# ACMMM2021-Anonymous/video-graph-ssl

Hardware: AMD Instinct MI355X
Metric: pretrain_clips_per_sec (higher is better)
Workload: dtype bf16x6 (fp32 tensors; conv products as 6 bf16 MFMAs on hi/mid/lo splits = fp32-grade, fp32 accumulate; everything else fp32)

## Files before the change

### include/gca_hip.h

```cpp
#ifndef GCA_HIP_H
#define GCA_HIP_H

#include <stdint.h>

#ifdef __cplusplus
extern "C" {
#endif

#define GCA_OK 0
#define GCA_EINVAL (-1)
#define GCA_ELAUNCH (-2)

int gca_version(void);

int gca_conv_halo_occupancy(int tm, int tn, int math, int64_t lds_bytes);

int gca_set_conv_math(int mode);
int gca_get_conv_math(void);

typedef struct {
  int32_t N, C, D, H, W;
  int32_t K;
  int32_t kd, kh, kw;
  int32_t sd, sh, sw;
// ... 64 lines not shown
                    float* save_mean, float* save_invstd, float* scale, float* shift, void* stream);
int gca_conv_fwd_slabs(const gca_conv_geom* g, const void* x, const float* wpack, const int32_t* table, void* ws,
                       int32_t* out_splits, void* stream);
int gca_bn_train_fwd_slabs(const float* slabs, int64_t splits, double count, const float* gamma, const float* beta, float eps,
                           float momentum, float* running_mean, float* running_var, int64_t* num_batches_tracked,
                           float* save_mean, float* save_invstd, float* scale, float* shift, float* y, const float* residual,
                           int relu, int64_t N, int64_t C, int64_t SP, float* z, int64_t z_batch_stride, void* stream);
int gca_bn_train_fwd(const float* stat_sum, const float* stat_sq, int64_t P, int64_t C, double count,
                     const float* gamma, const float* beta, float eps, float momentum,
                     float* running_mean, float* running_var, int64_t* num_batches_tracked,
                     float* save_mean, float* save_invstd, float* scale, float* shift,
                     const void* x, const void* residual, int relu, int64_t N, int64_t SP, void* z,
                     int64_t z_batch_stride, int act_f16, void* stream);
int gca_bn_fold_eval(const float* gamma, const float* beta, const float* running_mean,
                     const float* running_var, float eps, int64_t C, float* scale, float* shift, void* stream);
int gca_bn_apply(const void* x, const float* scale, const float* shift, const void* residual,
                 int relu, int64_t N, int64_t C, int64_t SP, void* z, int64_t z_batch_stride, int act_f16, void* stream);
int64_t gca_bn_bwd_ws_bytes(int64_t N, int64_t C, int64_t SP);
int gca_bn_bwd(const void* dz_in, const void* z, const void* x, const float* gamma,
               const float* save_mean, const float* save_invstd, int relu,
               int64_t N, int64_t C, int64_t SP, void* dx, float* dgamma, float* dbeta,
               void* dres, int dres_accumulate, int64_t z_batch_stride ,
               const float* scale, const float* shift, void* ws, int act_f16, void* stream);

typedef struct {
  int32_t N, C, D, H, W;
  int32_t kd, kh, kw, sd, sh, sw, pd, ph, pw;
  int32_t OD, OH, OW;
} gca_pool_geom;
int gca_maxpool3d_fwd(const gca_pool_geom* g, const void* x, void* y, int32_t* argmax, const float* scale,
                      const float* shift, int act_f16, void* stream);
int gca_maxpool3d_bwd(const gca_pool_geom* g, const void* dy, const int32_t* argmax, void* dx,
                      int accumulate, int act_f16, void* stream);
int gca_avgpool3d_fwd(const gca_pool_geom* g, const float* x, float* y, void* stream);
int gca_avgpool3d_bwd(const gca_pool_geom* g, const float* dy, float* dx, int accumulate, void* stream);
int gca_wavgpool_fwd(const void* x, const float* wt, float norm, int64_t NC, int64_t D, int64_t HW,
                     float* y, int x_f16, void* stream);
int gca_wavgpool_bwd(const float* dy, const float* wt, float norm, int64_t NC, int64_t D, int64_t HW,
                     void* dx, int x_f16, void* stream);

int gca_relu_fwd(const float* x, int64_t n, float* y, void* stream);
int gca_relu_bwd(const float* dy, const float* y, int64_t n, float* dx, void* stream);
int gca_l2norm_fwd(const float* x, int64_t rows, int64_t dim, float eps, float* y, float* inv_norm, void* stream);
int gca_l2norm_bwd(const float* dy, const float* y, const float* inv_norm, int64_t rows, int64_t dim,
                   float* dx, void* stream);
int gca_negcos_fwd_bwd(const float* p, const float* z, int64_t rows, int64_t dim, float scale,
                       float* loss, int accumulate, float* dp, void* stream);

int64_t gca_infonce_ws_bytes(int64_t b, int64_t K);
int gca_moco_logits_fwd(const float* q, const float* k, const float* queue, int64_t b, int64_t K,
                        int64_t D, float inv_T, float* logits, float* row_lse, int32_t* rank_ge, float* loss,
                        void* ws, uint32_t* sync_counter, void* stream);
int gca_nce_softmax_loss_fwd(const float* logits, int64_t b, int64_t ncol, const float* row_lse_in,
                             float* row_lse_out, float* loss, void* stream);
int gca_nce_softmax_loss_bwd(const float* logits, const float* row_lse, int64_t b, int64_t ncol,
                             const float* gscale_dev, float gscale_host, float* dlogits, void* stream);
int gca_moco_logits_bwd(const float* dlogits, const float* logits, const float* row_lse,
                        const float* gscale_dev, float gscale_host,
                        const float* k, const float* queue, int64_t b, int64_t K, int64_t D, float inv_T,
                        int64_t ov_start, const int64_t* ov_start_dev ,
                        int64_t ov_n, const float* ov_rows, float* dq, void* ws, void* stream);
int gca_rank_ge(const float* output, const int64_t* target, int64_t b, int64_t ncol, int32_t* rank_ge, void* stream);
int gca_queue_enqueue(float* queue, int64_t K, int64_t D, const float* keys, int64_t n, int64_t ptr,
                      const int64_t* ptr_dev, float* saved_rows, void* stream);
int gca_queue_advance(int64_t* ptr_dev, int64_t n, int64_t K, void* stream);

// ... 39 lines not shown
```

### video-graph-ssl_amd/_hip.py

```python
import ctypes as C
import os

import torch

_HERE = os.path.dirname(os.path.abspath(__file__))
LIB_PATH = os.environ.get('GCA_LIB_PATH') or os.path.join(_HERE, 'libgca_hip.so')


class HipLibraryMissing(RuntimeError):
    pass


if not os.path.exists(LIB_PATH):
    raise HipLibraryMissing(
        'libgca_hip.so is not built (%s). Run ./build_hip.sh or __graft_entry__.build(); there is no '
        'CPU fallback for the product path.' % LIB_PATH)
lib = C.CDLL(LIB_PATH)

c_i32, c_i64, c_f32, c_f64, c_vp = C.c_int32, C.c_int64, C.c_float, C.c_double, C.c_void_p


class ConvGeom(C.Structure):
    _fields_ = [(n, c_i32) for n in ('N', 'C', 'D', 'H', 'W', 'K', 'kd', 'kh', 'kw', 'sd', 'sh', 'sw',
                                     'pd', 'ph', 'pw', 'OD', 'OH', 'OW')] + [('x_batch_stride', c_i64)] + \
# ... 12 lines not shown
SIGNATURES = {
    'gca_version': (c_i32, []),
    'gca_conv_halo_occupancy': (c_i32, [c_i32, c_i32, c_i32, c_i64]),
    'gca_set_conv_math': (c_i32, [c_i32]),
    'gca_get_conv_math': (c_i32, []),
    'gca_conv_pack_elems': (c_i64, [_GP, c_i32]),
    'gca_conv_pack': (c_i32, [_GP, c_i32, c_vp, c_vp, c_vp]),
    'gca_conv_table_rows': (c_i64, [_GP, c_i32]),
    'gca_conv_table_build_host': (c_i32, [_GP, c_i32, c_vp]),
    'gca_conv_fwd_stat_parts': (c_i64, [_GP]),
    'gca_conv_kernel_cfg': (c_i32, [_GP, c_i32, c_vp]),
    'gca_conv_pack_layout': (c_i64, [_GP, c_i32]),
    'gca_conv_fwd_ws_bytes': (c_i64, [_GP]),
    'gca_conv_fwd': (c_i32, [_GP, c_vp, c_vp, c_vp, c_vp, c_vp, c_vp, c_vp, c_vp, c_vp]),
    'gca_conv_dgrad_ws_bytes': (c_i64, [_GP]),
    'gca_conv_dgrad': (c_i32, [_GP, c_vp, c_vp, c_vp, c_vp, c_i32, c_vp, c_vp]),
    'gca_conv_wgrad_cfg': (c_i32, [_GP, c_vp]),
    'gca_conv_wgrad_ws_bytes': (c_i64, [_GP]),
    'gca_conv_wgrad': (c_i32, [_GP, c_vp, c_vp, c_vp, c_vp, c_i32, c_vp, c_vp]),
    'gca_bias_grad': (c_i32, [c_vp, c_i64, c_i64, c_i64, c_vp, c_i32, c_vp]),
    'gca_bn_stats': (c_i32, [c_vp, c_i64, c_i64, c_i64, c_vp, c_vp, c_vp, c_i32, c_vp]),
    'gca_bn_stats_parts': (c_i64, [c_i64, c_i64, c_i64]),
    'gca_bn_finalize': (c_i32, [c_vp, c_vp, c_i64, c_i64, c_f64, c_vp, c_vp, c_f32, c_f32, c_vp, c_vp, c_vp,
                                c_vp, c_vp, c_vp, c_vp, c_vp]),
    'gca_bn_train_fwd': (c_i32, [c_vp, c_vp, c_i64, c_i64, c_f64, c_vp, c_vp, c_f32, c_f32, c_vp, c_vp, c_vp,
                                 c_vp, c_vp, c_vp, c_vp, c_vp, c_vp, c_i32, c_i64, c_i64, c_vp, c_i64, c_i32, c_vp]),
    'gca_bn_fold_eval': (c_i32, [c_vp, c_vp, c_vp, c_vp, c_f32, c_i64, c_vp, c_vp, c_vp]),
    'gca_bn_apply': (c_i32, [c_vp, c_vp, c_vp, c_vp, c_i32, c_i64, c_i64, c_i64, c_vp, c_i64, c_i32, c_vp]),
    'gca_bn_bwd_ws_bytes': (c_i64, [c_i64, c_i64, c_i64]),
    'gca_bn_bwd': (c_i32, [c_vp, c_vp, c_vp, c_vp, c_vp, c_vp, c_i32, c_i64, c_i64, c_i64, c_vp, c_vp, c_vp,
                           c_vp, c_i32, c_i64, c_vp, c_vp, c_vp, c_i32, c_vp]),
    'gca_maxpool3d_fwd': (c_i32, [_PP, c_vp, c_vp, c_vp, c_vp, c_vp, c_i32, c_vp]),
    'gca_maxpool3d_bwd': (c_i32, [_PP, c_vp, c_vp, c_vp, c_i32, c_i32, c_vp]),
    'gca_avgpool3d_fwd': (c_i32, [_PP, c_vp, c_vp, c_vp]),
    'gca_avgpool3d_bwd': (c_i32, [_PP, c_vp, c_vp, c_i32, c_vp]),
    'gca_wavgpool_fwd': (c_i32, [c_vp, c_vp, c_f32, c_i64, c_i64, c_i64, c_vp, c_i32, c_vp]),
    'gca_wavgpool_bwd': (c_i32, [c_vp, c_vp, c_f32, c_i64, c_i64, c_i64, c_vp, c_i32, c_vp]),
    'gca_relu_fwd': (c_i32, [c_vp, c_i64, c_vp, c_vp]),
    'gca_relu_bwd': (c_i32, [c_vp, c_vp, c_i64, c_vp, c_vp]),
    'gca_l2norm_fwd': (c_i32, [c_vp, c_i64, c_i64, c_f32, c_vp, c_vp, c_vp]),
    'gca_l2norm_bwd': (c_i32, [c_vp, c_vp, c_vp, c_i64, c_i64, c_vp, c_vp]),
    'gca_negcos_fwd_bwd': (c_i32, [c_vp, c_vp, c_i64, c_i64, c_f32, c_vp, c_i32, c_vp, c_vp]),
    'gca_infonce_ws_bytes': (c_i64, [c_i64, c_i64]),
    'gca_moco_logits_fwd': (c_i32, [c_vp, c_vp, c_vp, c_i64, c_i64, c_i64, c_f32, c_vp, c_vp, c_vp, c_vp, c_vp, c_vp, c_vp]),
    'gca_nce_softmax_loss_fwd': (c_i32, [c_vp, c_i64, c_i64, c_vp, c_vp, c_vp, c_vp]),
    'gca_nce_softmax_loss_bwd': (c_i32, [c_vp, c_vp, c_i64, c_i64, c_vp, c_f32, c_vp, c_vp]),
    'gca_moco_logits_bwd': (c_i32, [c_vp, c_vp, c_vp, c_vp, c_f32, c_vp, c_vp, c_i64, c_i64, c_i64, c_f32,
                                    c_i64, c_vp, c_i64, c_vp, c_vp, c_vp, c_vp]),
    'gca_queue_enqueue': (c_i32, [c_vp, c_i64, c_i64, c_vp, c_i64, c_i64, c_vp, c_vp, c_vp]),
    'gca_queue_advance': (c_i32, [c_vp, c_i64, c_i64, c_vp]),
    'gca_graph_gram_ws_bytes': (c_i64, [c_i64, c_i64, c_i64, c_i64]),
    'gca_graph_adj_fwd': (c_i32, [c_vp, c_vp, c_i64, c_i64, c_i64, c_i64, c_i32, c_f32, c_f32, c_vp, c_vp,
                                  c_vp, c_vp, c_vp, c_vp]),
    'gca_graph_adj_bwd': (c_i32, [c_vp, c_vp, c_vp, c_vp, c_vp, c_vp, c_i64, c_i64, c_i64, c_i64, c_i32, c_f32,
                                  c_f32, c_vp, c_vp, c_vp]),
    'gca_graph_gcn_fwd': (c_i32, [c_vp, c_vp, c_i64, c_i64, c_i64, c_i64, c_vp, c_vp]),
    'gca_graph_gcn_bwd_ws_bytes': (c_i64, [c_i64, c_i64, c_i64, c_i64]),
    'gca_graph_gcn_bwd': (c_i32, [c_vp, c_vp, c_vp, c_i64, c_i64, c_i64, c_i64, c_vp, c_vp, c_vp, c_vp]),
    'gca_ema_update': (c_i32, [c_vp, c_vp, c_i64, c_f32, c_vp]),
    'gca_sgd_step': (c_i32, [c_vp, c_vp, c_vp, c_i64, c_vp, c_vp, c_f32, c_f32, c_i32, c_i32, c_vp, c_vp]),
    'gca_grad_clip_ws_bytes': (c_i64, []),
    'gca_grad_clip_coef': (c_i32, [c_vp, c_i64, c_f32, c_vp, c_vp, c_vp]),
    'gca_conv_wgrad_partial': (c_i32, [_GP, c_vp, c_vp, c_vp, c_vp, c_vp, c_vp, c_vp, c_vp]),
    'gca_conv_xf_ok': (c_i32, [_GP]),
    'gca_conv_fwd_xf': (c_i32, [_GP, c_vp, c_vp, c_vp, c_vp, c_vp, c_vp, c_vp, c_vp, c_vp, c_vp, c_vp]),
    'gca_conv_wgrad_xf': (c_i32, [_GP, c_vp, c_vp, c_vp, c_vp, c_vp, c_vp, c_i32, c_vp, c_vp]),
# ... 65 lines not shown
```

### video-graph-ssl_amd/csrc/bn.hip

```cpp
#include "gca_common.h"

namespace {

constexpr int STAT_CHUNK = 8192;
constexpr int MAX_PARTS = 256;
constexpr long long BN_SMALL_ELEMS = 32768;

__host__ __device__ inline long long stats_parts(long long N, long long C, long long SP) {
  long long p = (N * SP + STAT_CHUNK - 1) / STAT_CHUNK;
  if (p < 1) p = 1;
  if (p > MAX_PARTS) p = MAX_PARTS;
  return p;
}

template <typename T, int MODE, int VEC>
__global__ __launch_bounds__(256) void bn_reduce_kernel(
    const T* __restrict__ a, const T* __restrict__ z, const T* __restrict__ x,
    const float* __restrict__ mean, const float* __restrict__ invstd, int relu,
    long long N, long long C, long long SP, long long zs, int P, float* __restrict__ out0,
    float* __restrict__ out1, const float* __restrict__ scale, const float* __restrict__ shift) {
  typedef gca_act<T> A_;
  __shared__ double sh[4];
  const int c = blockIdx.y, part = blockIdx.x;
  const float rsc = relu == 2 ? scale[c] : 0.f, rsf = relu == 2 ? shift[c] : 0.f;
// ... 588 lines not shown
                    (((uintptr_t)dz_in | (uintptr_t)z | (uintptr_t)x | (uintptr_t)dx | (uintptr_t)dres) % 16 == 0);
    if (s4)
      hipLaunchKernelGGL((bn_bwd_small_kernel<T, 4>), dim3((unsigned)C), dim3(256), 0, st, dz_in, z, x, gamma, save_mean, save_invstd,
                         relu, (int)N, (int)C, (int)SP, zs, dx, dgamma, dbeta, dres, dres_accumulate, scale, shift);
    else
      hipLaunchKernelGGL((bn_bwd_small_kernel<T, 1>), dim3((unsigned)C), dim3(256), 0, st, dz_in, z, x, gamma, save_mean, save_invstd,
                         relu, (int)N, (int)C, (int)SP, zs, dx, dgamma, dbeta, dres, dres_accumulate, scale, shift);
    return gca_launch_status();
  }
  const int P = (int)stats_parts(N, C, SP);
  float* p0 = reinterpret_cast<float*>(ws);
  float* p1 = p0 + (long long)C * P;
  float* coef = p1 + (long long)C * P;
  if ((SP % 4 == 0) && (zs % 4 == 0) && (((uintptr_t)dz_in | (uintptr_t)z | (uintptr_t)x) % 16 == 0))
    hipLaunchKernelGGL((bn_reduce_kernel<T, 1, 4>), dim3(P, (unsigned)C), dim3(256), 0, st, dz_in, z, x, save_mean,
                       save_invstd, relu, (long long)N, (long long)C, (long long)SP, zs, P, p0, p1, scale, shift);
  else
    hipLaunchKernelGGL((bn_reduce_kernel<T, 1, 1>), dim3(P, (unsigned)C), dim3(256), 0, st, dz_in, z, x, save_mean,
                       save_invstd, relu, (long long)N, (long long)C, (long long)SP, zs, P, p0, p1, scale, shift);
  hipLaunchKernelGGL(bn_bwd_finalize_kernel, dim3((unsigned)C), dim3(256), 0, st, p0, p1, P, (double)N * (double)SP,
                     gamma, save_invstd, dgamma, dbeta, coef, (long long)C);
  const long long total = (long long)N * C * SP;
  const bool v4 = (SP % 4 == 0) && (zs % 4 == 0) &&
                  (((uintptr_t)dz_in | (uintptr_t)z | (uintptr_t)x | (uintptr_t)dx | (uintptr_t)dres) % 16 == 0);
  if (v4)
    hipLaunchKernelGGL((bn_bwd_apply_kernel<T, 4>), dim3(ew_grid(total, 4)), dim3(256), 0, st, dz_in, z, x, save_mean,
                       save_invstd, coef, relu, total, (long long)C, (long long)SP, zs, dx, dres, dres_accumulate, scale, shift);
  else
    hipLaunchKernelGGL((bn_bwd_apply_kernel<T, 1>), dim3(ew_grid(total, 1)), dim3(256), 0, st, dz_in, z, x, save_mean,
                       save_invstd, coef, relu, total, (long long)C, (long long)SP, zs, dx, dres, dres_accumulate, scale, shift);
  return gca_launch_status();
}

extern "C" {

int64_t gca_bn_stats_parts(int64_t N, int64_t C, int64_t SP) { return stats_parts(N, C, SP); }


int gca_bn_finalize(const float* stat_sum, const float* stat_sq, int64_t P, int64_t C, double count,
                    const float* gamma, const float* beta, float eps, float momentum,
                    float* running_mean, float* running_var, int64_t* num_batches_tracked,
                    float* save_mean, float* save_invstd, float* scale, float* shift, void* stream) {
  if (!stat_sum || !stat_sq || P <= 0 || C <= 0 || count <= 0 || !scale || !shift) return GCA_EINVAL;
  hipLaunchKernelGGL(bn_finalize_kernel, dim3((unsigned)C), dim3(256), 0, (hipStream_t)stream, stat_sum, stat_sq,
                     (long long)P, count, gamma, beta, eps, momentum, running_mean, running_var, save_mean,
                     save_invstd, scale, shift, (long long*)num_batches_tracked);
  return gca_launch_status();
}


int gca_bn_fold_eval(const float* gamma, const float* beta, const float* running_mean,
                     const float* running_var, float eps, int64_t C, float* scale, float* shift, void* stream) {
  if (!running_mean || !running_var || !scale || !shift || C <= 0) return GCA_EINVAL;
  hipLaunchKernelGGL(bn_fold_eval_kernel, dim3((unsigned)gca_ceil_div(C, 256)), dim3(256), 0, (hipStream_t)stream,
                     gamma, beta, running_mean, running_var, eps, (long long)C, scale, shift);
  return gca_launch_status();
}


int64_t gca_bn_bwd_ws_bytes(int64_t N, int64_t C, int64_t SP) {
  if (N <= 0 || C <= 0 || SP <= 0) return GCA_EINVAL;
  return (int64_t)sizeof(float) * (2 * C * stats_parts(N, C, SP) + 3 * C);
}


int gca_bn_stats(const void* x, int64_t N, int64_t C, int64_t SP, float* stat_sum, float* stat_sq,
// ... 58 lines not shown
```

### video-graph-ssl_amd/csrc/gca_common.h

```cpp
#pragma once
#include <hip/hip_runtime.h>
#include <stdint.h>
#include "../../include/gca_hip.h"

#define GCA_WAVE 64

static inline int gca_launch_status() {
  hipError_t e = hipGetLastError();
  return e == hipSuccess ? GCA_OK : GCA_ELAUNCH;
}

static inline int64_t gca_ceil_div(int64_t a, int64_t b) { return (a + b - 1) / b; }
static inline int64_t gca_round_up(int64_t a, int64_t b) { return gca_ceil_div(a, b) * b; }

struct gca_magic { unsigned m; int s; unsigned d; };
static inline gca_magic gca_make_magic(unsigned d) {
  gca_magic g{0u, 0, d};
  if (d <= 1) return g;
  int s = 0;
  while ((1ull << s) < d) ++s;
  g.s = s;
  g.m = (unsigned)((((1ull << s) - d) << 32) / d + 1);
  return g;
}
// ... 34 lines not shown
  __syncthreads();
  return sh[0] + sh[1] + sh[2] + sh[3];
}
__device__ __forceinline__ double gca_block_sum256_d(double v, double* sh) {
  v = gca_wave_sum_d(v);
  const int w = threadIdx.x >> 6;
  __syncthreads();
  if ((threadIdx.x & 63) == 0) sh[w] = v;
  __syncthreads();
  return sh[0] + sh[1] + sh[2] + sh[3];
}

typedef _Float16 gca_half;
template <typename T> struct gca_act;
template <> struct gca_act<float> {
  static __device__ __forceinline__ float ld(const float* p) { return *p; }
  static __device__ __forceinline__ void st(float* p, float v) { *p = v; }
  static __device__ __forceinline__ float4 ld4(const float* p) { return *reinterpret_cast<const float4*>(p); }
  static __device__ __forceinline__ void st4(float* p, float4 v) { *reinterpret_cast<float4*>(p) = v; }
};
template <> struct gca_act<gca_half> {
  typedef _Float16 h4 __attribute__((ext_vector_type(4)));
  static __device__ __forceinline__ float ld(const gca_half* p) { return (float)*p; }
  static __device__ __forceinline__ void st(gca_half* p, float v) { *p = (gca_half)v; }
  static __device__ __forceinline__ float4 ld4(const gca_half* p) {
    const h4 v = *reinterpret_cast<const h4*>(p);
    return make_float4((float)v.x, (float)v.y, (float)v.z, (float)v.w);
  }
  static __device__ __forceinline__ void st4(gca_half* p, float4 v) {
    h4 o; o.x = (gca_half)v.x; o.y = (gca_half)v.y; o.z = (gca_half)v.z; o.w = (gca_half)v.w;
    *reinterpret_cast<h4*>(p) = o;
  }
};
```

### video-graph-ssl_amd/csrc/pool.hip

```cpp
#include "gca_common.h"
#include <math.h>
#include <cstdlib>

namespace {

struct PoolMagic {
  gca_magic osp, ohw, ow;
  gca_magic sp, hw, w;
  gca_magic sd, sh, sw;
  gca_magic c;
};

template <typename T, int KD, int KH, int KW>
__global__ __launch_bounds__(256) void maxpool3d_fwd_kernel(gca_pool_geom g, PoolMagic q, const T* __restrict__ x,
                                                            T* __restrict__ y, int* __restrict__ argmax,
                                                            unsigned total, const float* __restrict__ scale,
                                                            const float* __restrict__ shift) {
  const unsigned i = blockIdx.x * 256u + threadIdx.x;
  if (i >= total) return;
  const unsigned plane = gca_fdiv(i, q.osp), o = i - plane * q.osp.d;
  float sc = 1.f, sf = 0.f;
  if (scale) { const unsigned c = plane - gca_fdiv(plane, q.c) * q.c.d; sc = scale[c]; sf = shift[c]; }
#define GCA_POOL_VAL(v) (scale ? fmaxf((v) * sc + sf, 0.f) : (v))
  const int od = (int)gca_fdiv(o, q.ohw), r = (int)(o - (unsigned)od * q.ohw.d);
// ... 117 lines not shown
  const int OHW = g.OH * g.OW;
  const long long obase = (long long)plane * ((long long)g.OD * OHW);
  float acc = 0.f;
  if (CD > 0) {
    constexpr int NE = CD * CH * CW > 0 ? CD * CH * CW : 1;
    int am[NE];
    float gv[NE];
    bool okv[NE];
#pragma unroll
    for (int a = 0; a < CD; ++a)
#pragma unroll
      for (int b = 0; b < CH; ++b)
#pragma unroll
        for (int c = 0; c < CW; ++c) {
          const int od = od_lo + a, oh = oh_lo + b, ow = ow_lo + c;
          const bool ok = od <= od_hi && oh <= oh_hi && ow <= ow_hi;
          const long long o = obase + (ok ? (long long)od * OHW + oh * g.OW + ow : 0);
          const int e = (a * CH + b) * CW + c;
          okv[e] = ok; am[e] = argmax[o]; gv[e] = (float)dy[o];
        }
#pragma unroll
    for (int e = 0; e < CD * CH * CW; ++e) acc += (okv[e] && am[e] == s) ? gv[e] : 0.f;
  } else {
    for (int od = od_lo; od <= od_hi; ++od)
      for (int oh = oh_lo; oh <= oh_hi; ++oh)
        for (int ow = ow_lo; ow <= ow_hi; ++ow) {
          const long long o = obase + (long long)od * OHW + oh * g.OW + ow;
          if (argmax[o] == s) acc += (float)dy[o];
        }
  }
  dx[i] = (T)(accumulate ? (float)dx[i] + acc : acc);
}

template <typename T>
__global__ __launch_bounds__(256) void maxpool3d_bwd_brick333s2_kernel(gca_pool_geom g, gca_magic msp, gca_magic mhw, gca_magic mw,
                                                                       const T* __restrict__ dy, const int* __restrict__ argmax,
                                                                       T* __restrict__ dx, unsigned nbricks, int accumulate) {
  const unsigned t = blockIdx.x * 256u + threadIdx.x;
  if (t >= nbricks) return;
  const unsigned plane = gca_fdiv(t, msp), sidx = t - plane * msp.d;
  const int n = (int)gca_fdiv(sidx, mhw), r = (int)(sidx - (unsigned)n * mhw.d);
  const int m = (int)gca_fdiv((unsigned)r, mw), j = r - m * (int)mw.d;
  const bool vd1 = n + 1 < g.OD, vh1 = m + 1 < g.OH, vw2 = 2 * j + 2 < g.OW;
  const unsigned o00 = ((plane * (unsigned)g.OD + (unsigned)n) * (unsigned)g.OH + (unsigned)m) * (unsigned)g.OW + 2u * (unsigned)j;
  const unsigned step_d = vd1 ? (unsigned)(g.OH * g.OW) : 0u, step_h = vh1 ? (unsigned)g.OW : 0u, step_w = vw2 ? 2u : 1u;
  int2 a01[4];
  int a2[4];
  float g0[4], g1[4], g2[4];
#pragma unroll
  for (int c = 0; c < 4; ++c) {
    const unsigned o = o00 + ((c & 2) ? step_d : 0u) + ((c & 1) ? step_h : 0u);
    a01[c] = *reinterpret_cast<const int2*>(argmax + o);
    a2[c] = argmax[o + step_w];
    if (sizeof(T) == 4) {
      const float2 v = *reinterpret_cast<const float2*>(dy + o);
      g0[c] = v.x; g1[c] = v.y;
    } else {
      typedef _Float16 h2 __attribute__((ext_vector_type(2)));
      const h2 v = *reinterpret_cast<const h2*>(dy + o);
      g0[c] = (float)v.x; g1[c] = (float)v.y;
    }
    g2[c] = (float)dy[o + step_w];
  }
  if (!vw2) { a2[0] = a2[1] = a2[2] = a2[3] = -1; }
  if (!vd1) { a01[2] = a01[3] = make_int2(-1, -1); a2[2] = a2[3] = -1; }
  if (!vh1) { a01[1] = a01[3] = make_int2(-1, -1); a2[1] = a2[3] = -1; }
  const unsigned plane_base = plane * (unsigned)(g.D * g.H * g.W);
#pragma unroll
  for (int dd = 0; dd < 2; ++dd)
#pragma unroll
    for (int hh = 0; hh < 2; ++hh) {
      const int d = 2 * n + dd, h = 2 * m + hh;
      if (d >= g.D || h >= g.H) continue;
      const int s0 = (d * g.H + h) * g.W + 4 * j;
      float acc[4] = {0.f, 0.f, 0.f, 0.f};
#pragma unroll
      for (int cd = 0; cd <= dd; ++cd)
#pragma unroll
        for (int ch = 0; ch <= hh; ++ch) {
          const int c = 2 * cd + ch;
          acc[0] += a01[c].x == s0 ? g0[c] : 0.f;
          acc[1] += a01[c].x == s0 + 1 ? g0[c] : 0.f;
          acc[1] += a01[c].y == s0 + 1 ? g1[c] : 0.f;
          acc[2] += a01[c].y == s0 + 2 ? g1[c] : 0.f;
          acc[3] += a01[c].y == s0 + 3 ? g1[c] : 0.f;
          acc[3] += a2[c] == s0 + 3 ? g2[c] : 0.f;
        }
      T* out = dx + (plane_base + (unsigned)s0);
      if (accumulate) {
        const float4 o = gca_act<T>::ld4(out);
        acc[0] += o.x; acc[1] += o.y; acc[2] += o.z; acc[3] += o.w;
      }
      gca_act<T>::st4(out, make_float4(acc[0], acc[1], acc[2], acc[3]));
    }
}

template <typename T>
__global__ __launch_bounds__(256) void wavgpool_fwd_kernel(const T* __restrict__ x, const float* __restrict__ wt,
                                                           float norm, long long NC, int D, int HW,
                                                           float* __restrict__ y) {
  const long long p = (long long)blockIdx.x * 4 + (threadIdx.x >> 6);
  if (p >= NC) return;
  const int lane = threadIdx.x & 63;
  const T* xp = x + p * ((long long)D * HW);
  float s = 0.f;
  for (int d = 0; d < D; ++d) {
    float t = 0.f;
    for (int i = lane; i < HW; i += 64) t += (float)xp[(long long)d * HW + i];
    s += (wt ? wt[d] : 1.f) * t;
  }
  s = gca_wave_sum(s);
  if (lane == 0) y[p] = s * norm;
}

template <typename T>
__global__ __launch_bounds__(256) void wavgpool_bwd_kernel(const float* __restrict__ dy, const float* __restrict__ wt,
                                                           float norm, long long total, int D, int HW,
                                                           T* __restrict__ dx) {
  const long long i = (long long)blockIdx.x * 256 + threadIdx.x;
  if (i >= total) return;
  const long long p = i / ((long long)D * HW);
  const int d = (int)((i / HW) % D);
  dx[i] = (T)(dy[p] * norm * (wt ? wt[d] : 1.f));
}

inline bool pool_ok(const gca_pool_geom* g) {
  if (!g || g->N <= 0 || g->C <= 0 || g->D <= 0 || g->H <= 0 || g->W <= 0) return false;
// ... 108 lines not shown
  do {                                                                                                                     \
    if (act_f16)                                                                                                           \
      hipLaunchKernelGGL((maxpool3d_bwd_kernel<gca_half, CD, CH, CW>), grid, dim3(256), 0, st, *g, q, (const gca_half*)dy, \
                         argmax, (gca_half*)dx, (unsigned)total, accumulate ? 1 : 0);                                      \
    else                                                                                                                   \
      hipLaunchKernelGGL((maxpool3d_bwd_kernel<float, CD, CH, CW>), grid, dim3(256), 0, st, *g, q, (const float*)dy,       \
                         argmax, (float*)dx, (unsigned)total, accumulate ? 1 : 0);                                         \
  } while (0)
  if (g->kd == 3 && g->kh == 3 && g->kw == 3 && g->sd == 2 && g->sh == 2 && g->sw == 2 && g->pd == 1 && g->ph == 1 && g->pw == 1 &&
      g->W % 4 == 0 && ((uintptr_t)dx % (act_f16 ? 8 : 16)) == 0 && ((uintptr_t)dy % (act_f16 ? 4 : 8)) == 0 &&
      ((uintptr_t)argmax % 8) == 0 && pool_tiled_on()) {
    const int d2 = (g->D + 1) / 2, h2 = (g->H + 1) / 2, w4 = g->W / 4;
    const unsigned nbricks = (unsigned)((long long)g->N * g->C * d2 * h2 * w4);
    const gca_magic msp = gca_make_magic((unsigned)(d2 * h2 * w4)), mhw = gca_make_magic((unsigned)(h2 * w4)),
                    mw = gca_make_magic((unsigned)w4);
    const dim3 bgrid((unsigned)gca_ceil_div((long long)nbricks, 256));
    if (act_f16)
      hipLaunchKernelGGL(maxpool3d_bwd_brick333s2_kernel<gca_half>, bgrid, dim3(256), 0, st, *g, msp, mhw, mw, (const gca_half*)dy,
                         argmax, (gca_half*)dx, nbricks, accumulate ? 1 : 0);
    else
      hipLaunchKernelGGL(maxpool3d_bwd_brick333s2_kernel<float>, bgrid, dim3(256), 0, st, *g, msp, mhw, mw, (const float*)dy,
                         argmax, (float*)dx, nbricks, accumulate ? 1 : 0);
    return gca_launch_status();
  }
  if (cd == 2 && ch == 2 && cw == 2) GCA_POOL_BWD(2, 2, 2);
  else if (cd == 1 && ch == 2 && cw == 2) GCA_POOL_BWD(1, 2, 2);
  else if (cd == 3 && ch == 3 && cw == 3) GCA_POOL_BWD(3, 3, 3);
  else if (cd == 1 && ch == 1 && cw == 1) GCA_POOL_BWD(1, 1, 1);
  else GCA_POOL_BWD(0, 0, 0);
#undef GCA_POOL_BWD
  return gca_launch_status();
}

static bool avgpool_ok(const gca_pool_geom* g) {
  return pool_ok(g) && g->sd == g->kd && g->sh == g->kh && g->sw == g->kw && g->pd == 0 && g->ph == 0 && g->pw == 0;
}
int gca_avgpool3d_fwd(const gca_pool_geom* g, const float* x, float* y, void* stream) {
  if (!avgpool_ok(g) || !x || !y) return GCA_EINVAL;
  const long long total = (long long)g->N * g->C * g->OD * g->OH * g->OW;
  if (total >= (1LL << 31) || (long long)g->D * g->H * g->W >= (1LL << 31)) return GCA_EINVAL;
  hipLaunchKernelGGL(avgpool3d_fwd_kernel, dim3((unsigned)gca_ceil_div(total, 256)), dim3(256), 0, (hipStream_t)stream, *g,
                     pool_magic(g), x, y, (unsigned)total);
  return gca_launch_status();
}
int gca_avgpool3d_bwd(const gca_pool_geom* g, const float* dy, float* dx, int accumulate, void* stream) {
  if (!avgpool_ok(g) || !dy || !dx) return GCA_EINVAL;
  const long long total = (long long)g->N * g->C * g->D * g->H * g->W;
  if (total >= (1LL << 31)) return GCA_EINVAL;
  hipLaunchKernelGGL(avgpool3d_bwd_kernel, dim3((unsigned)gca_ceil_div(total, 256)), dim3(256), 0, (hipStream_t)stream, *g,
                     pool_magic(g), dy, dx, (unsigned)total, accumulate ? 1 : 0);
  return gca_launch_status();
}

int gca_wavgpool_fwd(const void* x, const float* wt, float norm, int64_t NC, int64_t D, int64_t HW,
                     float* y, int x_f16, void* stream) {
  if (!x || !y || NC <= 0 || D <= 0 || HW <= 0) return GCA_EINVAL;
  if (x_f16)
    hipLaunchKernelGGL(wavgpool_fwd_kernel<gca_half>, dim3((unsigned)gca_ceil_div(NC, 4)), dim3(256), 0, (hipStream_t)stream,
                       (const gca_half*)x, wt, norm, (long long)NC, (int)D, (int)HW, y);
  else
    hipLaunchKernelGGL(wavgpool_fwd_kernel<float>, dim3((unsigned)gca_ceil_div(NC, 4)), dim3(256), 0, (hipStream_t)stream,
                       (const float*)x, wt, norm, (long long)NC, (int)D, (int)HW, y);
  return gca_launch_status();
}

int gca_wavgpool_bwd(const float* dy, const float* wt, float norm, int64_t NC, int64_t D, int64_t HW,
// ... 14 lines not shown
```

### video-graph-ssl_amd/engine/layers.py

```python
import math

import torch
import torch.nn as nn

from . import ops
from . import tape as _tape
from .tape import LazyVar, Var


GRAD_LOG = None


def _grad_of(p):
    if p.grad is None:
        p.grad = torch.zeros_like(p.data)
    if GRAD_LOG is not None:
        GRAD_LOG.append((_tape.CURRENT[0], p))
    return p.grad


class _PackedWeight(object):

    def _init_pack(self):
        self._pack, self._pack_plan, self._prepacked = [None, None], [None, None], [False, False]
# ... 342 lines not shown
    def back():
        if xv.needs_grad:
            xv.add_grad(ops.relu_bwd(yv.grad, y))
        yv.grad = None
    tape.record(back)
    return yv


def f_conv_bn_relu_maxpool(tape, conv, bn, pool, xv):
    plan, x, xf = _conv_input(conv, xv)
    N, K, OD, OH, OW = plan.out_shape
    SP = OD * OH * OW
    wp = conv.packed(plan, 0)
    if bn.training:
        if xf is not None:
            y, (ss, sq) = ops.conv_fwd_xf(plan, x, xf[0], xf[1], wp, stats=True)
        else:
            y, (ss, sq) = ops.conv_fwd(plan, x, wp, None, stats=True, w_raw=conv.weight.data)
        mean, invstd, scale, shift = _bn_scale_shift(bn, ss, sq, N * SP)
    else:
        if xf is not None:
            x, xf = _stored(xv.t), None
        y = ops.conv_fwd(plan, x, wp, None, w_raw=conv.weight.data)
        mean = invstd = None
        scale, shift = ops.bn_fold_eval(bn.weight.data, bn.bias.data, bn.running_mean, bn.running_var, bn.eps)
    pplan = ops.pool_plan(tuple(y.shape), pool.kernel_size, pool.stride, pool.padding)
    p, am = ops.maxpool_fwd(pplan, y, want_argmax=tape.recording, scale=scale, shift=shift)
    pv = Var(p, tape.recording)
    if tape.recording:
        if mean is None:
            raise NotImplementedError('backward through eval-mode BatchNorm is not on the pre-training path')

        def back():
            dz = ops.maxpool_bwd(pplan, pv.grad, am)
            pv.grad = None
            dy = ops.bn_bwd(dz, None, y, bn.weight.data, mean, invstd, 2, N, K, SP, _grad_of(bn.weight), _grad_of(bn.bias),
                            None, False, scale, shift)
            del dz
            ops.conv_wgrad(plan, x, dy, _grad_of(conv.weight), accumulate=True, xf=xf)
            if xv.needs_grad:
                buf, acc = xv.grad_buffer()
                ops.conv_dgrad(plan, dy, conv.packed(plan, 1), buf, acc, w_raw=conv.weight.data)
        tape.record(back)
    return pv


def f_maxpool(tape, pool, xv):
    x = xv.t
    plan = ops.pool_plan(tuple(x.shape), pool.kernel_size, pool.stride, pool.padding)
    y, am = ops.maxpool_fwd(plan, x, want_argmax=tape.recording and xv.needs_grad)
    yv = Var(y, tape.recording)

    def back():
        if xv.needs_grad:
            buf, acc = xv.grad_buffer()
            ops.maxpool_bwd(plan, yv.grad, am, buf, acc)
        yv.grad = None
    tape.record(back)
    return yv


def f_avgpool(tape, pool, xv):
    x = xv.t
    plan = ops.pool_plan(tuple(x.shape), pool.kernel_size, pool.stride, pool.padding)
    yv = Var(ops.avgpool_fwd(plan, x), tape.recording)

    def back():
        if xv.needs_grad:
            buf, acc = xv.grad_buffer()
            ops.avgpool_bwd(plan, yv.grad, buf, acc)
        yv.grad = None
# ... 79 lines not shown
```

### video-graph-ssl_amd/engine/ops.py

```python
import ctypes as C
import functools
import os

import torch

from .. import _hip as H
from .._hip import aptr, is_half, ptr, stream

F32 = torch.float32
F16 = torch.float16


def _t3(v):
    return (v, v, v) if isinstance(v, int) else tuple(int(a) for a in v)


class _Workspace:

    def __init__(self):
        self.buf = {}
        self.captured = set()
        self.retired = []

    def get(self, nbytes, device):
# ... 605 lines not shown

class PoolPlan:
    def __init__(self, x_shape, k, s, p):
        N, Cc, D, Hh, W = x_shape
        kd, kh, kw = _t3(k)
        sd, sh, sw = _t3(s)
        pd, ph, pw = _t3(p)
        OD, OH, OW = (D + 2 * pd - kd) // sd + 1, (Hh + 2 * ph - kh) // sh + 1, (W + 2 * pw - kw) // sw + 1
        self.g = H.PoolGeom(N, Cc, D, Hh, W, kd, kh, kw, sd, sh, sw, pd, ph, pw, OD, OH, OW)
        self.gp = C.byref(self.g)
        self.in_shape, self.out_shape = tuple(x_shape), (N, Cc, OD, OH, OW)


@functools.lru_cache(maxsize=None)
def pool_plan(x_shape, k, s, p):
    return PoolPlan(x_shape, k, s, p)


def maxpool_fwd(plan, x, want_argmax=True, scale=None, shift=None):
    y = torch.empty(plan.out_shape, dtype=x.dtype, device=x.device)
    am = torch.empty(plan.out_shape, dtype=torch.int32, device=x.device) if want_argmax else None
    H.call('gca_maxpool3d_fwd', plan.gp, aptr(x), aptr(y), ptr(am), ptr(scale), ptr(shift), is_half(x), stream())
    return y, am


def maxpool_bwd(plan, dy, argmax, dx=None, accumulate=False):
    if dx is None:
        dx = torch.empty(plan.in_shape, dtype=dy.dtype, device=dy.device)
        accumulate = False
    H.call('gca_maxpool3d_bwd', plan.gp, aptr(dy), ptr(argmax), aptr(dx), int(accumulate), is_half(dy, dx), stream())
    return dx


def avgpool_fwd(plan, x):
    y = torch.empty(plan.out_shape, dtype=F32, device=x.device)
    H.call('gca_avgpool3d_fwd', plan.gp, ptr(x), ptr(y), stream())
    return y


def avgpool_bwd(plan, dy, dx=None, accumulate=False):
    if dx is None:
        dx = torch.empty(plan.in_shape, dtype=F32, device=dy.device)
        accumulate = False
    H.call('gca_avgpool3d_bwd', plan.gp, ptr(dy), ptr(dx), int(accumulate), stream())
    return dx


def wavgpool_fwd(x, wt, norm):
    N, Cc, D, Hh, W = x.shape
    y = torch.empty((N, Cc), dtype=F32, device=x.device)
    H.call('gca_wavgpool_fwd', aptr(x), ptr(wt), float(norm), N * Cc, D, Hh * W, ptr(y), is_half(x), stream())
    return y


def wavgpool_bwd(dy, wt, norm, x_shape, dtype=F32):
    N, Cc, D, Hh, W = x_shape
    dx = torch.empty(x_shape, dtype=dtype, device=dy.device)
    H.call('gca_wavgpool_bwd', ptr(dy), ptr(wt), float(norm), N * Cc, D, Hh * W, aptr(dx), is_half(dx), stream())
    return dx


def relu_fwd(x):
    y = torch.empty_like(x)
    H.call('gca_relu_fwd', ptr(x), x.numel(), ptr(y), stream())
    return y

# ... 198 lines not shown
```

Before: 1629.

## Fuse maxpool backward into BatchNorm backward for stride-2 3x3x3 pools

Adds a fused path that recomputes the maxpool gradient scatter on the fly, first in a per-channel reduction kernel that forms the BN backward sums, then in an apply kernel that writes the conv-input gradient directly. The intermediate dz tensor is no longer materialized, saving a full write and re-read of the pre-pool gradient. In exchange, the argmax and dp reads are done twice, once per pass, and the sums kernel uses a channel-major access pattern with gathered brick loads. It is enabled by default through an environment flag and only applies to fp32 tensors with this pool geometry.

```diff
diff --git a/include/gca_hip.h b/include/gca_hip.h
--- a/include/gca_hip.h
+++ b/include/gca_hip.h
@@ -120,6 +120,10 @@
                       const float* shift, int act_f16, void* stream);
 int gca_maxpool3d_bwd(const gca_pool_geom* g, const void* dy, const int32_t* argmax, void* dx,
                       int accumulate, int act_f16, void* stream);
+int64_t gca_bn_bwd_maxpool_ws_bytes(const gca_pool_geom* g);
+int gca_bn_bwd_maxpool(const gca_pool_geom* g, const float* dp, const int32_t* argmax, const float* y, const float* gamma,
+                       const float* save_mean, const float* save_invstd, const float* scale, const float* shift, float* dy,
+                       float* dgamma, float* dbeta, void* ws, void* stream);
 int gca_avgpool3d_fwd(const gca_pool_geom* g, const float* x, float* y, void* stream);
 int gca_avgpool3d_bwd(const gca_pool_geom* g, const float* dy, float* dx, int accumulate, void* stream);
 int gca_wavgpool_fwd(const void* x, const float* wt, float norm, int64_t NC, int64_t D, int64_t HW,
diff --git a/video-graph-ssl_amd/_hip.py b/video-graph-ssl_amd/_hip.py
--- a/video-graph-ssl_amd/_hip.py
+++ b/video-graph-ssl_amd/_hip.py
@@ -68,6 +68,8 @@
                            c_vp, c_i32, c_i64, c_vp, c_vp, c_vp, c_i32, c_vp]),
     'gca_maxpool3d_fwd': (c_i32, [_PP, c_vp, c_vp, c_vp, c_vp, c_vp, c_i32, c_vp]),
     'gca_maxpool3d_bwd': (c_i32, [_PP, c_vp, c_vp, c_vp, c_i32, c_i32, c_vp]),
+    'gca_bn_bwd_maxpool_ws_bytes': (c_i64, [_PP]),
+    'gca_bn_bwd_maxpool': (c_i32, [_PP, c_vp, c_vp, c_vp, c_vp, c_vp, c_vp, c_vp, c_vp, c_vp, c_vp, c_vp, c_vp, c_vp]),
     'gca_avgpool3d_fwd': (c_i32, [_PP, c_vp, c_vp, c_vp]),
     'gca_avgpool3d_bwd': (c_i32, [_PP, c_vp, c_vp, c_i32, c_vp]),
     'gca_wavgpool_fwd': (c_i32, [c_vp, c_vp, c_f32, c_i64, c_i64, c_i64, c_vp, c_i32, c_vp]),
diff --git a/video-graph-ssl_amd/csrc/bn.hip b/video-graph-ssl_amd/csrc/bn.hip
--- a/video-graph-ssl_amd/csrc/bn.hip
+++ b/video-graph-ssl_amd/csrc/bn.hip
@@ -644,6 +644,13 @@
   return gca_launch_status();
 }
 
+int gca_bn_bwd_finalize_launch(const float* p0, const float* p1, int P, double count, const float* gamma, const float* invstd,
+                               float* dgamma, float* dbeta, float* coef, int64_t C, void* stream) {
+  hipLaunchKernelGGL(bn_bwd_finalize_kernel, dim3((unsigned)C), dim3(256), 0, (hipStream_t)stream, p0, p1, P, count, gamma, invstd,
+                     dgamma, dbeta, coef, (long long)C);
+  return gca_launch_status();
+}
+
 extern "C" {
 
 int64_t gca_bn_stats_parts(int64_t N, int64_t C, int64_t SP) { return stats_parts(N, C, SP); }
diff --git a/video-graph-ssl_amd/csrc/gca_common.h b/video-graph-ssl_amd/csrc/gca_common.h
--- a/video-graph-ssl_amd/csrc/gca_common.h
+++ b/video-graph-ssl_amd/csrc/gca_common.h
@@ -90,3 +90,6 @@
     *reinterpret_cast<h4*>(p) = o;
   }
 };
+
+int gca_bn_bwd_finalize_launch(const float* p0, const float* p1, int P, double count, const float* gamma, const float* invstd,
+                               float* dgamma, float* dbeta, float* coef, int64_t C, void* stream);
diff --git a/video-graph-ssl_amd/csrc/pool.hip b/video-graph-ssl_amd/csrc/pool.hip
--- a/video-graph-ssl_amd/csrc/pool.hip
+++ b/video-graph-ssl_amd/csrc/pool.hip
@@ -173,6 +173,56 @@
   dx[i] = (T)(accumulate ? (float)dx[i] + acc : acc);
 }
 
+struct PoolBrick {
+  int2 a01[4];
+  int a2[4];
+  float g0[4], g1[4], g2[4];
+};
+
+template <typename T>
+__device__ __forceinline__ void pool_brick_fetch(const gca_pool_geom& g, unsigned plane, int n, int m, int j, const T* __restrict__ dy,
+                                                 const int* __restrict__ argmax, PoolBrick& b, bool want_d1 = true,
+                                                 bool want_h1 = true) {
+  const bool vd1 = want_d1 && n + 1 < g.OD, vh1 = want_h1 && m + 1 < g.OH, vw2 = 2 * j + 2 < g.OW;
+  const unsigned o00 = ((plane * (unsigned)g.OD + (unsigned)n) * (unsigned)g.OH + (unsigned)m) * (unsigned)g.OW + 2u * (unsigned)j;
+  const unsigned step_d = vd1 ? (unsigned)(g.OH * g.OW) : 0u, step_h = vh1 ? (unsigned)g.OW : 0u, step_w = vw2 ? 2u : 1u;
+#pragma unroll
+  for (int c = 0; c < 4; ++c) {
+    const unsigned o = o00 + ((c & 2) ? step_d : 0u) + ((c & 1) ? step_h : 0u);
+    b.a01[c] = *reinterpret_cast<const int2*>(argmax + o);
+    b.a2[c] = argmax[o + step_w];
+    if (sizeof(T) == 4) {
+      const float2 v = *reinterpret_cast<const float2*>(dy + o);
+      b.g0[c] = v.x; b.g1[c] = v.y;
+    } else {
+      typedef _Float16 h2 __attribute__((ext_vector_type(2)));
+      const h2 v = *reinterpret_cast<const h2*>(dy + o);
+      b.g0[c] = (float)v.x; b.g1[c] = (float)v.y;
+    }
+    b.g2[c] = (float)dy[o + step_w];
+  }
+  if (!vw2) { b.a2[0] = b.a2[1] = b.a2[2] = b.a2[3] = -1; }
+  if (!vd1) { b.a01[2] = b.a01[3] = make_int2(-1, -1); b.a2[2] = b.a2[3] = -1; }
+  if (!vh1) { b.a01[1] = b.a01[3] = make_int2(-1, -1); b.a2[1] = b.a2[3] = -1; }
+}
+
+__device__ __forceinline__ void pool_brick_quad(const PoolBrick& b, int dd, int hh, int s0, float (&acc)[4]) {
+  acc[0] = acc[1] = acc[2] = acc[3] = 0.f;
+#pragma unroll
+  for (int cd = 0; cd < 2; ++cd)
+#pragma unroll
+    for (int ch = 0; ch < 2; ++ch) {
+      if (cd > dd || ch > hh) continue;
+      const int c = 2 * cd + ch;
+      acc[0] += b.a01[c].x == s0 ? b.g0[c] : 0.f;
+      acc[1] += b.a01[c].x == s0 + 1 ? b.g0[c] : 0.f;
+      acc[1] += b.a01[c].y == s0 + 1 ? b.g1[c] : 0.f;
+      acc[2] += b.a01[c].y == s0 + 2 ? b.g1[c] : 0.f;
+      acc[3] += b.a01[c].y == s0 + 3 ? b.g1[c] : 0.f;
+      acc[3] += b.a2[c] == s0 + 3 ? b.g2[c] : 0.f;
+    }
+}
+
 template <typename T>
 __global__ __launch_bounds__(256) void maxpool3d_bwd_brick333s2_kernel(gca_pool_geom g, gca_magic msp, gca_magic mhw, gca_magic mw,
                                                                        const T* __restrict__ dy, const int* __restrict__ argmax,
@@ -182,30 +232,8 @@
   const unsigned plane = gca_fdiv(t, msp), sidx = t - plane * msp.d;
   const int n = (int)gca_fdiv(sidx, mhw), r = (int)(sidx - (unsigned)n * mhw.d);
   const int m = (int)gca_fdiv((unsigned)r, mw), j = r - m * (int)mw.d;
-  const bool vd1 = n + 1 < g.OD, vh1 = m + 1 < g.OH, vw2 = 2 * j + 2 < g.OW;
-  const unsigned o00 = ((plane * (unsigned)g.OD + (unsigned)n) * (unsigned)g.OH + (unsigned)m) * (unsigned)g.OW + 2u * (unsigned)j;
-  const unsigned step_d = vd1 ? (unsigned)(g.OH * g.OW) : 0u, step_h = vh1 ? (unsigned)g.OW : 0u, step_w = vw2 ? 2u : 1u;
-  int2 a01[4];
-  int a2[4];
-  float g0[4], g1[4], g2[4];
-#pragma unroll
-  for (int c = 0; c < 4; ++c) {
-    const unsigned o = o00 + ((c & 2) ? step_d : 0u) + ((c & 1) ? step_h : 0u);
-    a01[c] = *reinterpret_cast<const int2*>(argmax + o);
-    a2[c] = argmax[o + step_w];
-    if (sizeof(T) == 4) {
-      const float2 v = *reinterpret_cast<const float2*>(dy + o);
-      g0[c] = v.x; g1[c] = v.y;
-    } else {
-      typedef _Float16 h2 __attribute__((ext_vector_type(2)));
-      const h2 v = *reinterpret_cast<const h2*>(dy + o);
-      g0[c] = (float)v.x; g1[c] = (float)v.y;
-    }
-    g2[c] = (float)dy[o + step_w];
-  }
-  if (!vw2) { a2[0] = a2[1] = a2[2] = a2[3] = -1; }
-  if (!vd1) { a01[2] = a01[3] = make_int2(-1, -1); a2[2] = a2[3] = -1; }
-  if (!vh1) { a01[1] = a01[3] = make_int2(-1, -1); a2[1] = a2[3] = -1; }
+  PoolBrick b;
+  pool_brick_fetch<T>(g, plane, n, m, j, dy, argmax, b);
   const unsigned plane_base = plane * (unsigned)(g.D * g.H * g.W);
 #pragma unroll
   for (int dd = 0; dd < 2; ++dd)
@@ -214,19 +242,8 @@
       const int d = 2 * n + dd, h = 2 * m + hh;
       if (d >= g.D || h >= g.H) continue;
       const int s0 = (d * g.H + h) * g.W + 4 * j;
-      float acc[4] = {0.f, 0.f, 0.f, 0.f};
-#pragma unroll
-      for (int cd = 0; cd <= dd; ++cd)
-#pragma unroll
-        for (int ch = 0; ch <= hh; ++ch) {
-          const int c = 2 * cd + ch;
-          acc[0] += a01[c].x == s0 ? g0[c] : 0.f;
-          acc[1] += a01[c].x == s0 + 1 ? g0[c] : 0.f;
-          acc[1] += a01[c].y == s0 + 1 ? g1[c] : 0.f;
-          acc[2] += a01[c].y == s0 + 2 ? g1[c] : 0.f;
-          acc[3] += a01[c].y == s0 + 3 ? g1[c] : 0.f;
-          acc[3] += a2[c] == s0 + 3 ? g2[c] : 0.f;
-        }
+      float acc[4];
+      pool_brick_quad(b, dd, hh, s0, acc);
       T* out = dx + (plane_base + (unsigned)s0);
       if (accumulate) {
         const float4 o = gca_act<T>::ld4(out);
@@ -234,6 +251,98 @@
       }
       gca_act<T>::st4(out, make_float4(acc[0], acc[1], acc[2], acc[3]));
     }
+}
+
+__device__ __forceinline__ void pool_bn_bwd_brick(const gca_pool_geom& g, unsigned plane, unsigned sidx, gca_magic mhw, gca_magic mw,
+                                                  const float* __restrict__ dp, const int* __restrict__ argmax,
+                                                  const float* __restrict__ y, float rsc, float rsf, float mu, float is,
+                                                  float A, float B, float Cc, float* __restrict__ dy) {
+  const int n = (int)gca_fdiv(sidx, mhw), r = (int)(sidx - (unsigned)n * mhw.d);
+  const int m = (int)gca_fdiv((unsigned)r, mw), j = r - m * (int)mw.d;
+  PoolBrick b;
+  pool_brick_fetch<float>(g, plane, n, m, j, dp, argmax, b);
+  const unsigned plane_base = plane * (unsigned)(g.D * g.H * g.W);
+  float4 yv[4];
+  int s0[4];
+#pragma unroll
+  for (int q = 0; q < 4; ++q) {
+    const int d = min(2 * n + (q >> 1), g.D - 1), h = min(2 * m + (q & 1), g.H - 1);
+    s0[q] = (d * g.H + h) * g.W + 4 * j;
+    yv[q] = *reinterpret_cast<const float4*>(y + (plane_base + (unsigned)s0[q]));
+  }
+#pragma unroll
+  for (int q = 0; q < 4; ++q) {
+    if (2 * n + (q >> 1) >= g.D || 2 * m + (q & 1) >= g.H) continue;
+    float acc[4];
+    pool_brick_quad(b, q >> 1, q & 1, s0[q], acc);
+    const float xe[4] = {yv[q].x, yv[q].y, yv[q].z, yv[q].w};
+    float o[4];
+#pragma unroll
+    for (int e = 0; e < 4; ++e) {
+      float dz = acc[e];
+      if (!(xe[e] * rsc + rsf > 0.f)) dz = 0.f;
+      o[e] = A * (dz - B - (xe[e] - mu) * is * Cc);
+    }
+    *reinterpret_cast<float4*>(dy + (plane_base + (unsigned)s0[q])) = make_float4(o[0], o[1], o[2], o[3]);
+  }
+}
+
+__global__ __launch_bounds__(256) void pool_bn_bwd_sums_333s2_kernel(
+    gca_pool_geom g, gca_magic msp, gca_magic mhw, gca_magic mw, unsigned M, unsigned per, int P, const float* __restrict__ dp,
+    const int* __restrict__ argmax, const float* __restrict__ y, const float* __restrict__ scale, const float* __restrict__ shift,
+    const float* __restrict__ mean, const float* __restrict__ invstd, float* __restrict__ out0, float* __restrict__ out1) {
+  __shared__ double sh[4];
+  const unsigned c = blockIdx.y, part = blockIdx.x;
+  const float rsc = scale[c], rsf = shift[c], mu = mean[c], is = invstd[c];
+  const unsigned lo = part * per, hi = min(lo + per, M);
+  double s0 = 0.0, s1 = 0.0;
+  auto group = [&](unsigned i, float4& dz, float4& xv) __attribute__((always_inline)) {
+    const unsigned n = gca_fdiv(i, msp), sp = i - n * msp.d;
+    const unsigned d = gca_fdiv(sp, mhw), r = sp - d * mhw.d, h = gca_fdiv(r, mw), j = (r - h * mw.d) >> 2;
+    const unsigned plane = n * (unsigned)g.C + c;
+    PoolBrick b;
+    pool_brick_fetch<float>(g, plane, (int)(d >> 1), (int)(h >> 1), (int)j, dp, argmax, b, (d & 1u) != 0, (h & 1u) != 0);
+    float acc[4];
+    pool_brick_quad(b, 1, 1, (int)sp, acc);
+    dz = make_float4(acc[0], acc[1], acc[2], acc[3]);
+    xv = *reinterpret_cast<const float4*>(y + (plane * msp.d + sp));
+  };
+  auto accum = [&](const float4 dv, const float4 xv) __attribute__((always_inline)) {
+    const float dzq[4] = {dv.x, dv.y, dv.z, dv.w}, xe[4] = {xv.x, xv.y, xv.z, xv.w};
+#pragma unroll
+    for (int e = 0; e < 4; ++e) {
+      float dz = dzq[e];
+      if (!(xe[e] * rsc + rsf > 0.f)) dz = 0.f;
+      s0 += (double)dz; s1 += (double)dz * (double)((xe[e] - mu) * is);
+    }
+  };
+  for (unsigned i = lo + 4u * threadIdx.x; i < hi; i += 2048u) {
+    const unsigned i2 = i + 1024u;
+    const bool two = i2 < hi;
+    float4 dz0, dz1, x0, x1;
+    group(i, dz0, x0);
+    group(two ? i2 : i, dz1, x1);
+    accum(dz0, x0);
+    if (two) accum(dz1, x1);
+  }
+  s0 = gca_block_sum256_d(s0, sh);
+  s1 = gca_block_sum256_d(s1, sh);
+  if (threadIdx.x == 0) {
+    out0[(long long)c * P + part] = (float)s0;
+    out1[(long long)c * P + part] = (float)s1;
+  }
+}
+
+__global__ __launch_bounds__(256) void pool_bn_bwd_apply_brick333s2_kernel(
+    gca_pool_geom g, gca_magic msp, gca_magic mhw, gca_magic mw, gca_magic mc, unsigned nbricks, const float* __restrict__ dp,
+    const int* __restrict__ argmax, const float* __restrict__ y, const float* __restrict__ scale, const float* __restrict__ shift,
+    const float* __restrict__ mean, const float* __restrict__ invstd, const float* __restrict__ coef, float* __restrict__ dy) {
+  const unsigned t = blockIdx.x * 256u + threadIdx.x;
+  if (t >= nbricks) return;
+  const unsigned plane = gca_fdiv(t, msp), sidx = t - plane * msp.d;
+  const unsigned c = plane - gca_fdiv(plane, mc) * mc.d;
+  pool_bn_bwd_brick(g, plane, sidx, mhw, mw, dp, argmax, y, scale[c], shift[c], mean[c], invstd[c], coef[c], coef[g.C + c],
+                          coef[2 * g.C + c], dy);
 }
 
 template <typename T>
@@ -408,6 +517,41 @@
   return gca_launch_status();
 }
 
+static bool pool_brick_form(const gca_pool_geom* g) {
+  return pool_ok(g) && g->kd == 3 && g->kh == 3 && g->kw == 3 && g->sd == 2 && g->sh == 2 && g->sw == 2 && g->pd == 1 && g->ph == 1 &&
+         g->pw == 1 && g->W % 4 == 0 && (long long)g->N * g->C * g->D * g->H * g->W < (1LL << 31);
+}
+int64_t gca_bn_bwd_maxpool_ws_bytes(const gca_pool_geom* g) {
+  if (!pool_brick_form(g)) return GCA_EINVAL;
+  return gca_bn_bwd_ws_bytes(g->N, g->C, (int64_t)g->D * g->H * g->W);
+}
+
+int gca_bn_bwd_maxpool(const gca_pool_geom* g, const float* dp, const int32_t* argmax, const float* y, const float* gamma,
+                       const float* save_mean, const float* save_invstd, const float* scale, const float* shift, float* dy,
+                       float* dgamma, float* dbeta, void* ws, void* stream) {
+  if (!pool_brick_form(g) || !dp || !argmax || !y || !save_mean || !save_invstd || !scale || !shift || !dy || !ws) return GCA_EINVAL;
+  if (((uintptr_t)y % 16) || ((uintptr_t)dy % 16) || ((uintptr_t)dp % 8) || ((uintptr_t)argmax % 8) || ((uintptr_t)ws % 4)) return GCA_EINVAL;
+  const int d2 = (g->D + 1) / 2, h2 = (g->H + 1) / 2, w4 = g->W / 4;
+  const unsigned bpp = (unsigned)(d2 * h2 * w4), nbricks = (unsigned)((long long)g->N * g->C * bpp);
+  const long long SP = (long long)g->D * g->H * g->W, M = (long long)g->N * SP;
+  const int P = (int)gca_bn_stats_parts(g->N, g->C, SP);
+  const long long per = ((M + P - 1) / P + 3) & ~3LL;
+  const gca_magic msp = gca_make_magic(bpp), mhw = gca_make_magic((unsigned)(h2 * w4)), mw = gca_make_magic((unsigned)w4),
+                  mc = gca_make_magic((unsigned)g->C), esp = gca_make_magic((unsigned)SP),
+                  ehw = gca_make_magic((unsigned)(g->H * g->W)), ew = gca_make_magic((unsigned)g->W);
+  float* p0 = reinterpret_cast<float*>(ws);
+  float* p1 = p0 + (long long)g->C * P;
+  float* coef = p1 + (long long)g->C * P;
+  hipStream_t st = (hipStream_t)stream;
+  hipLaunchKernelGGL(pool_bn_bwd_sums_333s2_kernel, dim3((unsigned)P, (unsigned)g->C), dim3(256), 0, st, *g, esp, ehw, ew, (unsigned)M,
+                     (unsigned)per, P, dp, argmax, y, scale, shift, save_mean, save_invstd, p0, p1);
+  const int rc = gca_bn_bwd_finalize_launch(p0, p1, P, (double)g->N * (double)SP, gamma, save_invstd, dgamma, dbeta, coef, g->C, stream);
+  if (rc) return rc;
+  hipLaunchKernelGGL(pool_bn_bwd_apply_brick333s2_kernel, dim3((unsigned)gca_ceil_div((long long)nbricks, 256)), dim3(256), 0, st, *g,
+                     msp, mhw, mw, mc, nbricks, dp, argmax, y, scale, shift, save_mean, save_invstd, coef, dy);
+  return gca_launch_status();
+}
+
 static bool avgpool_ok(const gca_pool_geom* g) {
   return pool_ok(g) && g->sd == g->kd && g->sh == g->kh && g->sw == g->kw && g->pd == 0 && g->ph == 0 && g->pw == 0;
 }
diff --git a/video-graph-ssl_amd/engine/layers.py b/video-graph-ssl_amd/engine/layers.py
--- a/video-graph-ssl_amd/engine/layers.py
+++ b/video-graph-ssl_amd/engine/layers.py
@@ -398,11 +398,16 @@
             raise NotImplementedError('backward through eval-mode BatchNorm is not on the pre-training path')
 
         def back():
-            dz = ops.maxpool_bwd(pplan, pv.grad, am)
-            pv.grad = None
-            dy = ops.bn_bwd(dz, None, y, bn.weight.data, mean, invstd, 2, N, K, SP, _grad_of(bn.weight), _grad_of(bn.bias),
-                            None, False, scale, shift)
-            del dz
+            if ops.FUSE_POOL_BN and ops.bn_bwd_maxpool_ok(pplan, pv.grad, y):
+                dy = ops.bn_bwd_maxpool(pplan, pv.grad, am, y, bn.weight.data, mean, invstd, scale, shift,
+                                        _grad_of(bn.weight), _grad_of(bn.bias))
+                pv.grad = None
+            else:
+                dz = ops.maxpool_bwd(pplan, pv.grad, am)
+                pv.grad = None
+                dy = ops.bn_bwd(dz, None, y, bn.weight.data, mean, invstd, 2, N, K, SP, _grad_of(bn.weight), _grad_of(bn.bias),
+                                None, False, scale, shift)
+                del dz
             ops.conv_wgrad(plan, x, dy, _grad_of(conv.weight), accumulate=True, xf=xf)
             if xv.needs_grad:
                 buf, acc = xv.grad_buffer()
diff --git a/video-graph-ssl_amd/engine/ops.py b/video-graph-ssl_amd/engine/ops.py
--- a/video-graph-ssl_amd/engine/ops.py
+++ b/video-graph-ssl_amd/engine/ops.py
@@ -661,6 +661,21 @@
     return dx
 
 
+FUSE_POOL_BN = os.environ.get('GCA_FUSE_POOL_BN', '1') != '0'
+
+
+def bn_bwd_maxpool_ok(plan, dp, y):
+    return dp.dtype is F32 and y.dtype is F32 and H.lib.gca_bn_bwd_maxpool_ws_bytes(plan.gp) > 0
+
+
+def bn_bwd_maxpool(plan, dp, argmax, y, gamma, mean, invstd, scale, shift, dgamma, dbeta):
+    dy = torch.empty_like(y)
+    ws = WS.get(H.lib.gca_bn_bwd_maxpool_ws_bytes(plan.gp), y.device)
+    H.call('gca_bn_bwd_maxpool', plan.gp, ptr(dp), ptr(argmax), ptr(y), ptr(gamma), ptr(mean), ptr(invstd), ptr(scale),
+           ptr(shift), ptr(dy), ptr(dgamma), ptr(dbeta), ptr(ws), stream())
+    return dy
+
+
 def avgpool_fwd(plan, x):
     y = torch.empty(plan.out_shape, dtype=F32, device=x.device)
     H.call('gca_avgpool3d_fwd', plan.gp, ptr(x), ptr(y), stream())
```

Result: no change. 1633, median of 2 (+0.2%).
